# solonas13/REAL

Measured on AMD Instinct MI355X. Metric: aligned reads/sec (100 bp, k≤3) at 1/2/4/8 MI355X; achieved HBM GB/s vs peak, higher is better.
Workload: dtype u64

## Files before the change

### real_amd/csrc/match_common.h

```cpp
#pragma once
#include "kernel_common.h"

template <int W>
__device__ __forceinline__ void revcomp_words(const uint64_t *in, uint64_t *out, uint32_t patl)
{
    const uint32_t nw = (patl + 31) >> 5;
    const uint32_t pad = 64 * nw - 2 * patl;
#pragma unroll
    for (int j = 0; j < W; ++j) {
        uint64_t x = 0, y = 0;
#pragma unroll
        for (int k = 0; k < W; ++k) {
            if ((uint32_t)k + (uint32_t)j + 1 == nw) x = rev2(in[k]);
            if ((uint32_t)k + (uint32_t)j + 2 == nw) y = rev2(in[k]);
        }
        const uint64_t v = pad ? ((x << pad) | (y >> (64 - pad))) : x;
        const uint64_t valid = ((uint32_t)j + 1 < nw) ? ~0ull : ((uint32_t)j + 1 == nw ? (~0ull << pad) : 0ull);
        out[j] = ~v & valid;
    }
}

struct LdsRow {
    const uint8_t *stg;
    uint32_t lb;
    __device__ __forceinline__ uint32_t dword(int byteoff, uint32_t) const
    {
        const uint32_t o = lb + (uint32_t)byteoff;
        const uint32_t *p = reinterpret_cast<const uint32_t *>(stg + (o & ~3u));
        return __builtin_amdgcn_alignbyte(p[1], p[0], o & 3u);
    }
};
struct GlobalRow {
    const uint8_t *row;
    __device__ __forceinline__ uint32_t dword(int byteoff, uint32_t patl) const
    {
        uint32_t v = 0;
#pragma unroll
        for (int b = 0; b < 4; ++b) {
            const int i = byteoff + b;
            if (i >= 0 && i < (int)patl) v |= (uint32_t)row[i] << (8 * b);
        }
        return v;
    }
};

template <int W, class Row>
__device__ __forceinline__ bool pack_read(const Row &row, uint32_t patl, uint64_t *O)
{
    bool ok = true;
#pragma unroll
    for (int j = 0; j < W; ++j) {
        uint64_t w = 0;
#pragma unroll
        for (int d = 0; d < 8; ++d) {
            const uint32_t bo = 32u * j + 4u * d;
            if (bo < patl) {
                uint32_t x = row.dword((int)bo, patl);
                const uint32_t rem = patl - bo;
                if (rem < 4) x &= (1u << (8 * rem)) - 1u;
                if (x & 0xfcfcfcfcu) ok = false;
                w |= (uint64_t)(((x & 0x03030303u) * 0x40100401u) >> 24) << (56 - 8 * d);
            }
        }
        O[j] = w;
    }
    return ok;
}

template <int W, class Row>
__device__ __forceinline__ void pack_read_packed(const Row &row, uint32_t patl, uint32_t skew, uint64_t *O)
{
    const uint32_t nbytes = (skew + patl + 3) >> 2;
    const uint32_t nw = (patl + 31) >> 5, sh = 2 * skew;
#pragma unroll
    for (int j = 0; j < W; ++j) {
        uint64_t w = 0;
        if ((uint32_t)j < nw) {
            const uint32_t hi = __builtin_bswap32(row.dword(8 * j, nbytes));
            const uint32_t lo = __builtin_bswap32(row.dword(8 * j + 4, nbytes));
            w = ((uint64_t)hi << 32) | lo;
            if (sh) w = (w << sh) | ((uint64_t)(row.dword(8 * j + 8, nbytes) & 0xffu) >> (8 - sh));
            const uint32_t rem = patl - 32u * j;
            if (rem < 32) w &= ~0ull << (64 - 2 * rem);
        }
        O[j] = w;
    }
}

template <int W>
__device__ __forceinline__ void seed_halves(const uint64_t *O, uint32_t l, uint64_t &shi, uint64_t &slo, uint64_t &rhi, uint64_t &rlo)
{
    const uint32_t h = l >> 1;
    const uint64_t hm = (h == 32) ? ~0ull : ((1ull << (2 * h)) - 1);
    shi = O[0] >> (64 - 2 * h);
    if (2 * h <= 32) slo = (O[0] >> (64 - 4 * h)) & hm;
    else slo = ((h == 32) ? O[W > 1 ? 1 : 0] : (((O[0] << (2 * h)) | (O[W > 1 ? 1 : 0] >> (64 - 2 * h))) >> (64 - 2 * h)));
    rhi = (rev2(slo) >> (64 - 2 * h)) ^ hm;
    rlo = (rev2(shi) >> (64 - 2 * h)) ^ hm;
}

#define RH_LL_ZERO 1024u
#define RH_LL_SLOTS 1025u
template <int W, class Row>
__device__ __forceinline__ float score_location(const double *sLL, const uint64_t *Ow, const uint64_t *tw, uint32_t patl,
                                                const Row &qrow, bool has_q, uint32_t inv)
{
    double raw = 1.0;
    constexpr int NQ = 2 * W;
    uint32_t th[NQ], oh[NQ];
#pragma unroll
    for (int c = 0; c < NQ; ++c) {
        th[c] = (uint32_t)(tw[c >> 1] >> ((c & 1) ? 0 : 32));
        oh[c] = (uint32_t)(Ow[c >> 1] >> ((c & 1) ? 0 : 32));
    }
    const uint32_t nchunk = (patl + 15) >> 4;
#pragma unroll 1
    for (uint32_t c = 0; c < nchunk; ++c) {
        uint32_t qa[4] = {0x1e1e1e1eu, 0x1e1e1e1eu, 0x1e1e1e1eu, 0x1e1e1e1eu};
        if (has_q) {
            if (!inv) {
#pragma unroll
                for (int i = 0; i < 4; ++i) qa[i] = qrow.dword((int)(16 * c) + 4 * i, patl);
            } else {
                const int p0 = (int)patl - 16 - (int)(16 * c);
#pragma unroll
                for (int i = 0; i < 4; ++i) qa[i] = __builtin_bswap32(qrow.dword(p0 + 4 * (3 - i), patl));
            }
        }
        const uint32_t lim = min(16u, patl - 16u * c);
        const uint32_t tr = th[0], rr = oh[0];
#pragma unroll
        for (int h = 0; h < 2; ++h) {
            double x[8];
#pragma unroll
            for (int v = 0; v < 8; ++v) {
                const uint32_t u = 8u * h + v;
                const uint32_t ref = (tr >> (30 - 2 * u)) & 3;
                const uint32_t rb = (rr >> (30 - 2 * u)) & 3;
                const uint32_t q = (qa[u >> 2] >> (8 * (u & 3))) & 0xff;
                const uint32_t idx = ((ref << 8) | (rb << 6) | q) & 1023;
                x[v] = sLL[u < lim ? idx : RH_LL_ZERO];
            }
#pragma unroll
            for (int v = 0; v < 8; ++v) raw += x[v];
        }
#pragma unroll
        for (int i = 0; i + 1 < NQ; ++i) { th[i] = th[i + 1]; oh[i] = oh[i + 1]; }
    }
    return (float)raw;
}

__device__ __forceinline__ float long_score(const double *sLL, const uint64_t *__restrict__ T, const uint64_t *cur, uint32_t pos, uint32_t patl,
                                            const uint8_t *qual, uint32_t inv)
{
    const uint64_t wi = pos >> 5;
    const unsigned sh = 2u * (pos & 31);
    const uint32_t nw = (patl + 31) >> 5;
    double raw = 1.0;
    uint64_t t0 = T[wi];
    for (uint32_t j = 0; j < nw; ++j) {
        const uint64_t t1 = T[wi + j + 1];
        const uint64_t al = sh ? ((t0 << sh) | (t1 >> (64 - sh))) : t0;
        const uint64_t rw = cur[j];
        const uint32_t nb = min(32u, patl - 32u * j);
        for (uint32_t u = 0; u < nb; ++u) {
            const uint32_t i = 32u * j + u;
            const uint32_t ref = (uint32_t)(al >> (62 - 2 * u)) & 3u, rb = (uint32_t)(rw >> (62 - 2 * u)) & 3u;
            const uint32_t q = qual ? (uint32_t)qual[inv ? patl - 1 - i : i] : 30u;
            raw += sLL[((ref << 8) | (rb << 6) | q) & 1023];
        }
        t0 = t1;
    }
    return (float)raw;
}
```

### real_amd/csrc/match_kernel.hip

```cpp
#include "match_common.h"
#include "row_bytes.h"
#include "complex_walk.h"

#ifndef RH_ABLATE
#define RH_ABLATE 0
#endif
#ifndef RH_PHASE_TIMING
#define RH_PHASE_TIMING 0
#endif

#ifndef RH_PHASE_SUB
#define RH_PHASE_SUB 0
#endif
#if RH_PHASE_TIMING
#define PH_NOW() ((unsigned)__builtin_amdgcn_s_memrealtime())
#define PH_SUB(N, DT) do { if (RH_PHASE_SUB == (N)) s.tD += (DT); else if (RH_PHASE_SUB == 4) s.tD -= (DT); } while (0)
#else
#define PH_NOW() 0u
#endif
#define EB 8
#define MQ 16
#define QUEUE_BYTES (MQ * 64u * 5u + 6u * 64u * 4u)
enum : int { TK_STARTS = 0, TK_DIRECTORY = 1, TK_ROWS = 3, TK_ROWS_WIDE = 4 };
__host__ __device__ constexpr uint32_t stg_bytes(int W, int TK) { return TK >= TK_ROWS ? 11008u : (W <= 4 ? QUEUE_BYTES : 9728u); }
// ... 932 lines not shown
    ISSUE_ROWS_P(0u);
#pragma unroll 1
    for (uint32_t li = 0; li < 6; ++li) {
        const uint32_t tbl = tbl_of(li);
        const bool pairt = li < 4;
#if RH_PHASE_TIMING
        const unsigned ph0 = PH_NOW();
#endif
        wave_lds_sync();
        {
            uint8_t *d = rowbuf + (lane >> 3) * 128 + (((lane & 7) ^ ((lane >> 3) & 7)) * 16);
            *reinterpret_cast<uint4 *>(d + 0 * 1024) = va0; *reinterpret_cast<uint4 *>(d + 1 * 1024) = va1;
            *reinterpret_cast<uint4 *>(d + 2 * 1024) = va2; *reinterpret_cast<uint4 *>(d + 3 * 1024) = va3;
            *reinterpret_cast<uint4 *>(d + 4 * 1024) = va4; *reinterpret_cast<uint4 *>(d + 5 * 1024) = va5;
            *reinterpret_cast<uint4 *>(d + 6 * 1024) = va6; *reinterpret_cast<uint4 *>(d + 7 * 1024) = va7;
        }
        wave_lds_sync();
#if RH_PHASE_TIMING
        unsigned ph1 = PH_NOW();
        s.tW += ph1 - ph0;
#endif
        const uint8_t *rowb = rowbuf + lane * 128;
        const uint32_t sw = lane & 7;
        auto row = [&](uint32_t d) { return *reinterpret_cast<const uint32_t *>(rowb + ((((d >> 2) ^ sw) << 4) | ((d & 3) << 2))); };
        auto row16 = [&](uint32_t B) { return (uint32_t)*reinterpret_cast<const uint16_t *>(rowb + rh_row_lds_byte(B, sw)); };
        const uint32_t g0 = rnext & 255u, g1 = (rnext >> 8) & 255u, s0 = rnext >> 16, la1 = pairt ? 5 - tbl : tbl;
        const uint32_t r0 = sig_of(s0, 5 - tbl) >> (a.l - pbits);
        const uint32_t r1 = sig_of(s0 ^ 1u, 5 - la1) >> (a.l - pbits);
        const bool mine = act && !(s.p_n == PEND_OVF) && !(RH_ABLATE & 8);
        const uint32_t h0 = row(0), h1 = row(1);
        const bool cplx = mine && rh_row_complex(h0, h1);
        uint32_t c0 = 0, c1 = 0, eb0 = 0, eb1 = 0;
        if (mine && !cplx) {
            const uint64_t hh = ((uint64_t)h1 << 32) | h0, ones = 0x1111111111111111ull;
            const uint64_t below0 = ones & ~(~0ull << (4 * g0));
            eb0 = nibble_dot(h0, (uint32_t)below0, nibble_dot(h1, (uint32_t)(below0 >> 32), 0u));
            c0 = (uint32_t)(hh >> (4 * g0)) & 15u;
            const uint64_t ext = (ones & ~(~0ull << (4 * g1))) ^ below0;
            eb1 = nibble_dot(h0, (uint32_t)ext, nibble_dot(h1, (uint32_t)(ext >> 32), eb0));
            c1 = (uint32_t)(hh >> (4 * g1)) & 15u;
            s.addL(2u);
            s.addC(c0 + c1);
            s.addP(c0 + c1);
            if (RH_ABLATE & 4) c0 = c1 = 0;
        }
        uint32_t xb0 = 0, xc0 = 0, xb1 = 0, xc1 = 0;
        bool inplace = false;
        if (__any(cplx)) {
            if (cplx) {
                const uint32_t w[4] = {row(4), row(5), row(6), row(7)};
                const uint32_t o0 = row(2), tot = row(3);
                CwGroup ga, gb;
                cw_header2(w, g0, g1, ga, gb);
                s.addL(1u);
                xb0 = o0 + ga.off; xc0 = ga.cnt;
                if (ga.sat) {
                    const uint2 kr = key_group_range(a.ix.ent[tbl], o0, o0 + tot, pbits, g0);
                    xb0 = kr.x; xc0 = kr.y;
                }
                s.addC(xc0);
                s.addP(xc0);
                if (xc0 > T::BIG) { s.p_n = PEND_OVF; s.cslot = xc0 <= BIG_T2 ? SLOT_NONE : SLOT_BIG; xc0 = 0; }
                else {
                    s.addL(1u);
                    xb1 = o0 + gb.off; xc1 = gb.cnt;
                    if (gb.sat) {
                        const uint2 kr = key_group_range(a.ix.ent[tbl], o0, o0 + tot, pbits, g1);
                        xb1 = kr.x; xc1 = kr.y;
                    }
                    s.addC(xc1);
                    s.addP(xc1);
                    if (xc1 > T::BIG) { s.p_n = PEND_OVF; s.cslot = xc1 <= BIG_T2 ? SLOT_NONE : SLOT_BIG; xc0 = xc1 = 0; }
                }
                if (RH_ABLATE & 4) xc0 = xc1 = 0;
            }
            const uint64_t m0 = __ballot(xc0 != 0), m1 = __ballot(xc1 != 0);
            const uint32_t n0 = (uint32_t)__popcll(m0), n1 = (uint32_t)__popcll(m1);
            inplace = cw_n + n0 + n1 > T::CWCAP;
            if (!inplace) {
                const uint32_t i0 = cw_n + __builtin_amdgcn_mbcnt_hi((uint32_t)(m0 >> 32), __builtin_amdgcn_mbcnt_lo((uint32_t)m0, 0u));
                const uint32_t i1 = cw_n + n0 + __builtin_amdgcn_mbcnt_hi((uint32_t)(m1 >> 32), __builtin_amdgcn_mbcnt_lo((uint32_t)m1, 0u));
                if (xc0) cwl[i0] = make_uint2(xb0, cw_pack(lane, xc0, tbl, tbl, s0));
                if (xc1) cwl[i1] = make_uint2(xb1, cw_pack(lane, xc1, tbl, la1, s0 ^ 1u));
                cw_n += n0 + n1;
                xc0 = xc1 = 0;
            }
        }
        const bool walk = li == 5 && cw_n != 0;
        uint32_t *cw_pre = bkx;
        uint32_t cw_total = 0;
        auto fetch = [&](uint32_t t, uint2 &e, uint32_t &m, uint32_t &k) {
            const bool ok = t < cw_total;
            const uint32_t d = cw_flat_find(cw_pre, cw_n, ok ? t : 0u);
            const uint2 ds = cwl[d];
            const uint32_t tb = cw_table(ds.y), own = cw_lane(ds.y), st = cw_strand(ds.y);
            const uint2 *E = tb == 0u ? a.ix.ent[0] : tb == 1u ? a.ix.ent[1] : tb == 2u ? a.ix.ent[2] : a.ix.ent[3];
            e = make_uint2(0u, 0u);
            if (ok) e = E[ds.x + (t - cw_pre[d])];
            m = ok ? ds.y : CW_NONE;
            const uint32_t ohf = __shfl(fhi, (int)own), olf = __shfl(flo, (int)own), ohr = __shfl(rhi, (int)own), olr = __shfl(rlo, (int)own);
            k = sig_from(st ? ohr : ohf, st ? olr : olf, 5u - cw_list(ds.y)) >> (a.l - pbits);
        };
        uint2 e_c = make_uint2(0u, 0u), e_n = make_uint2(0u, 0u);
        uint32_t m_c = CW_NONE, k_c = 0, m_n = CW_NONE, k_n = 0;
#if RH_PHASE_TIMING
        const unsigned pw0 = PH_NOW();
#endif
        if (walk) {
            static_assert(T::CWCAP * 4u <= 256u, "the prefix sums lie in the place of the bucket numbers");
            wave_lds_sync();
            const uint32_t cnt = lane < cw_n ? cw_cnt(cwl[lane].y) : 0u;
            uint32_t inc = cnt;
#pragma unroll
            for (uint32_t d = 1; d < 64; d <<= 1) {
                const uint32_t v = __shfl_up(inc, d);
                if (lane >= d) inc += v;
            }
            cw_total = __builtin_amdgcn_readlane(inc, 63);
            wave_lds_sync();
            if (lane < cw_n) cw_pre[lane] = inc - cnt;
            wave_lds_sync();
            fetch(lane, e_c, m_c, k_c);
            if (cw_total > 64u) fetch(64u + lane, e_n, m_n, k_n);
        }
#if RH_PHASE_TIMING
        const unsigned pw1 = PH_NOW();
#endif
        U64x2 pre = {0ull, 0ull};
        if (inplace && xc0) pre = load2(reinterpret_cast<const uint64_t *>(a.ix.ent[tbl] + xb0));
        if (li + 1 < 6) ISSUE_ROWS_P(li + 1);
#if RH_PHASE_TIMING
        const unsigned ps1 = PH_NOW();
        PH_SUB(1, (ps1 - ph1) - (pw1 - pw0));
#endif
        {
            static_assert(RH_ROW_CAP < 32 && 2 * 15 < 32, "one mask word for both groups of a simple row (one group taken twice: 2 x 15 entries)");
            const uint32_t ct = c0 + c1, d1 = eb1 - c0;
            uint32_t rk0 = r0 >> (pbits - p16), rk1 = r1 >> (pbits - p16);
            asm volatile("" : "+v"(rk0), "+v"(rk1));
            uint32_t passm = 0, e_j = 0;
            while (__any(e_j < ct)) {
                uint32_t key[4];
#pragma unroll
                for (uint32_t u = 0; u < 4; ++u) {
                    const uint32_t jj = e_j + u;
                    const uint32_t ej = jj + (jj >= c0 ? d1 : eb0);
                    key[u] = row16(rh_row_key_byte(ej < RH_ROW_CAP - 1u ? ej : RH_ROW_CAP - 1u));
                }
                asm volatile("" : "+v"(key[0]), "+v"(key[1]), "+v"(key[2]), "+v"(key[3]));
#pragma unroll
                for (uint32_t u = 0; u < 4; ++u) {
                    const uint32_t jj = e_j + u;
                    const uint32_t x = key[u] ^ (jj >= c0 ? rk1 : rk0);
                    passm |= ((jj < ct) & passes(x) ? 1u : 0u) << (jj & 31u);
                }
                e_j += 4;
            }
            const uint32_t low = (1u << c0) - 1u;
            if (__popc(passm & low) > NPEND || __popc(passm & ~low) > NPEND) { s.p_n = PEND_OVF; passm = 0; }
#if RH_PHASE_TIMING
            const unsigned ps2 = PH_NOW();
            PH_SUB(2, ps2 - ps1);
#endif
            while (__any(passm != 0)) {
                const bool step = passm != 0;
                const uint32_t jj = step ? (uint32_t)__ffs((int)passm) - 1u : 0u;
                passm &= passm - 1u;
                const bool sec = jj >= c0;
                const uint32_t ej = step ? jj + (sec ? d1 : eb0) : 0u;
                const uint32_t plo = row16(rh_row_pos_byte(ej, 0u)), phi = row16(rh_row_pos_byte(ej, 1u));
                take(step, plo | (phi << 16), s0 ^ (sec ? 1u : 0u), sec ? la1 : tbl);
            }
#if RH_PHASE_TIMING
            PH_SUB(3, PH_NOW() - ps2);
#endif
        }
        if (inplace) {
#pragma unroll 1
            for (uint32_t half = 0; half < 2; ++half) {
                const uint32_t strand = s0 ^ half, la = half ? la1 : tbl, r = half ? r1 : r0;
                const uint32_t e_base = half ? xb1 : xb0;
                e_cnt = s.p_n == PEND_OVF ? 0u : (half ? xc1 : xc0);
                const bool e_ovf = e_cnt != 0;
                if (half) pre = e_ovf ? load2(reinterpret_cast<const uint64_t *>(a.ix.ent[tbl] + e_base)) : U64x2{0ull, 0ull};
                auto take_ovf = [&](bool ok, uint2 e) { take(ok && passes((e.x & pmask) ^ r), e.y, strand, la); };
                if (__any(e_ovf)) {
                    take_ovf(e_cnt > 0, make_uint2((uint32_t)pre.a, (uint32_t)(pre.a >> 32)));
                    take_ovf(e_cnt > 1, make_uint2((uint32_t)pre.b, (uint32_t)(pre.b >> 32)));
                }
                uint32_t e_j = 2;
                while (__any(e_j < e_cnt)) {
                    uint2 e[T::OVN];
#pragma unroll
                    for (uint32_t u = 0; u < T::OVN; ++u) e[u] = (e_j + u < e_cnt) ? a.ix.ent[tbl][e_base + e_j + u] : make_uint2(0u, 0u);
#pragma unroll
                    for (uint32_t u = 0; u < T::OVN; ++u) take_ovf(e_j + u < e_cnt, e[u]);
                    e_j += T::OVN;
                }
            }
        }
        if (walk) {
            uint32_t *cw_slot = reinterpret_cast<uint32_t *>(rowbuf);
#pragma unroll 1
            for (uint32_t t0 = 0; t0 < cw_total; t0 += 64u) {
                bool pend = m_c != CW_NONE && passes((e_c.x & pmask) ^ k_c);
                const uint32_t own = cw_lane(m_c);
                while (__any(pend)) {
                    wave_lds_sync();
                    cw_slot[lane] = CW_NONE;
                    wave_lds_sync();
                    if (pend) atomicMin(cw_slot + own, lane);
                    wave_lds_sync();
                    const uint32_t from = cw_slot[lane];
                    const bool hit = from != CW_NONE;
                    const int src = (int)(hit ? from : lane);
                    const uint32_t pos = __shfl(e_c.y, src), tag = __shfl(m_c, src);
                    if (pend && cw_slot[own] == lane) pend = false;
                    take(hit, pos, cw_strand(tag), cw_list(tag));
                }
                e_c = e_n; m_c = m_n; k_c = k_n;
                m_n = CW_NONE;
                if (t0 + 128u < cw_total) fetch(t0 + 128u + lane, e_n, m_n, k_n);
            }
        }
#if RH_PHASE_TIMING
        if (RH_PHASE_SUB == 0 || RH_PHASE_SUB == 4) s.tD += PH_NOW() - ph1;
#endif
    }
    const uint32_t patl = act ? s.patl : 32u * T::W;
#pragma unroll 1
    for (uint32_t inv = 0; inv < 2; ++inv) {
        if (inv && act) {
            uint64_t R[T::W];
            revcomp_words<T::W>(s.O, R, patl);
#pragma unroll
            for (int j = 0; j < T::W; ++j) s.O[j] = R[j];
        }
        s.shi = inv ? rhi : fhi; s.slo = inv ? rlo : flo;
        s.reset_strand((int)inv);
        if (T::SCORES && inv) {
            const uint8_t *qsrc;
            uint32_t qbytes, qlate, qskew;
            if (quals_ahead<T>(a, s.o0, s.o1, qsrc, qbytes, qlate, qskew)) {
                wave_lds_sync();
                const uint32_t lds0 = __builtin_amdgcn_readfirstlane((uint32_t)(uintptr_t)(__attribute__((address_space(3))) uint8_t *)rowbuf);
                QUAL_DMA(qlate, lds0, qbytes - qlate, 9u)
                const uint32_t tail0 = qbytes & ~15u;
                if (lane < (qbytes & 15u)) rowbuf[tail0 - qlate + lane] = qsrc[tail0 + lane];
            }
        }
#if RH_PHASE_TIMING
        const unsigned ph2 = PH_NOW();
#endif
        if (s.p_n == PEND_OVF) qn = 0;
        auto next = [&](uint32_t k) { while (k < qn && (q_getl(k) >> 6) != inv) ++k; return k; };
        CandText<T::W> c0;
        uint32_t k = next(0u), rp0 = 0, la0 = 0;
        if (k < qn) { rp0 = q_getp(k); la0 = q_getl(k); cand_load(a, s, rp0, c0); }
        while (k < qn) {
            CandText<T::W> c1;
            const uint32_t k1 = next(k + 1);
            uint32_t rp1 = 0, la1 = 0;
            if (k1 < qn) { rp1 = q_getp(k1); la1 = q_getl(k1); cand_load(a, s, rp1, c1); }
            process_loaded(a, s, sLL, rp0, la0 & 63u, c0);
            c0 = c1; rp0 = rp1; la0 = la1; k = k1;
        }
#if RH_PHASE_TIMING
        s.tR += PH_NOW() - ph2;
#endif
    }
    if (T::SCORES) {
        const uint8_t *qsrc;
        uint32_t qbytes, qlate, qskew;
        if (quals_ahead<T>(a, s.o0, s.o1, qsrc, qbytes, qlate, qskew) && qlate) {
            wave_lds_sync();
            const uint32_t lds0 = __builtin_amdgcn_readfirstlane((uint32_t)(uintptr_t)(__attribute__((address_space(3))) uint8_t *)stg);
            QUAL_DMA(0u, lds0 + STG_PAD, qlate, 3u)
        }
    }
#undef QUAL_DMA
#undef ISSUE_ROWS_P
}

template <class T, int LA0, int LA1>
__device__ __forceinline__ void match_lists(const MatchArgs &a, LaneState<T> &s, const double *sLL, uint32_t *q_pos, uint8_t *q_la)
{
    if (T::DIR) { match_lists_directory<T, LA0, LA1>(a, s, sLL, q_pos, q_la); return; }
    uint32_t qn = 0;
    scan_lists<T, LA0, LA1>(a, s, q_pos, q_la, qn);
    for (uint32_t k = 0; k < qn && s.p_n != PEND_OVF; ++k)
        process_candidate(a, s, sLL, q_pos[k * 64], (uint32_t)q_la[k * 64]);
}

template <class T>
__device__ __forceinline__ void match_read(const MatchArgs &a, LaneState<T> &s, const double *sLL, uint8_t *stg, uint32_t *q_pos, uint8_t *q_la,
                                           bool act)
{
    const uint32_t patl = act ? s.patl : 32u * T::W;
    s.reset_read();
    uint64_t rhi = 0, rlo = 0;
    if (act) seed_halves<T::W>(s.O, a.l, s.shi, s.slo, rhi, rlo);
    else { s.shi = s.slo = 0; }
    if constexpr (T::PAIRED) { match_rows_paired<T>(a, s, sLL, stg, act, (uint32_t)rhi, (uint32_t)rlo); return; }
    for (int inv = 0; inv < 2; ++inv) {
        if constexpr (!T::ROWS) {
            if (s.p_n == PEND_OVF) break;
        }
        if (inv && act) {
            uint64_t R[T::W];
            revcomp_words<T::W>(s.O, R, patl);
#pragma unroll
            for (int j = 0; j < T::W; ++j) s.O[j] = R[j];
            s.shi = rhi; s.slo = rlo;
        }
        s.reset_strand(inv);
        const bool go = !T::ROWS || (act && !(s.p_n == PEND_OVF));
        if (!T::ALL && !T::SCORES) {
            if constexpr (T::ROWS) match_lists_rows<T, 0, 1>(a, s, sLL, stg, go, false);
            else match_lists<T, 0, 1>(a, s, sLL, q_pos, q_la);
            const unsigned st = (unsigned)(s.info >> ST_SHIFT), er = (unsigned)(s.info >> ER_SHIFT) & 15;
            if constexpr (T::ROWS) match_lists_rows<T, 1, 6>(a, s, sLL, stg, go && !(st == (unsigned)(inv ? ST_REVERSE : ST_STRAIGHT) && er == 0), false);
            else if (!(st == (unsigned)(inv ? ST_REVERSE : ST_STRAIGHT) && er == 0)) match_lists<T, 1, 6>(a, s, sLL, q_pos, q_la);
        } else if constexpr (T::ROWS) {
            match_lists_rows<T, 0, 6>(a, s, sLL, stg, go, !T::PASS2 && inv != 0);
        } else {
            match_lists<T, 0, 6>(a, s, sLL, q_pos, q_la);
        }
    }
}

template <int W, bool SCORES, bool ALL, int TK, bool PASS2>
__global__ __launch_bounds__(256) __attribute__((amdgpu_waves_per_eu(PASS2 ? 2 : (W <= 5 ? 3 : 2)))) void match_kernel(MatchArgs a_)
{
    using T = LaneInst<W, SCORES, ALL, TK, PASS2>;
    constexpr uint32_t STG = T::STG;
    static_assert(!PASS2 || T::HAS_PASS2, "the second pass exists for bucket rows with parked hits only");
    __shared__ double sLL[SCORES ? RH_LL_SLOTS : 1];
    __shared__ __attribute__((aligned(16))) uint8_t smem[4 * STG];
    if (SCORES) {
        for (int i = threadIdx.x; i < 1024; i += 256) sLL[i] = a_.LL[i];
        if (threadIdx.x == 0) sLL[RH_LL_ZERO] = 0.0;
        __syncthreads();
    }
    const uint64_t n_items = PASS2 ? (uint64_t)*a_.ovf_count : a_.b.n_reads;
    const uint64_t n_tiles = (n_items + 63) / 64;
    uint32_t *const tile_ctr = PASS2 ? a_.tile_ctr2 : a_.tile_ctr;
    uint32_t next_raw = 0;
    if ((threadIdx.x & 63) == 0) next_raw = atomicAdd(tile_ctr, 1u);
    while (true) {
    const uint64_t tile = (uint32_t)__builtin_amdgcn_readfirstlane((int)next_raw);
    if (tile >= n_tiles) break;
    if ((threadIdx.x & 63) == 0) next_raw = atomicAdd(tile_ctr, 1u);
    uint32_t tid = threadIdx.x;
    asm volatile("" : "+v"(tid));
    const __attribute__((address_space(4))) MatchArgs *pa = (const __attribute__((address_space(4))) MatchArgs *)__builtin_amdgcn_kernarg_segment_ptr();
    asm volatile("" : "+s"(pa));
    const MatchArgs &a = *(const MatchArgs *)pa;
    const uint32_t lane = tid & 63;
    uint8_t *stg = smem + (tid >> 6) * STG;
    uint32_t *q_pos = reinterpret_cast<uint32_t *>(stg) + lane;
    uint8_t *q_la = stg + MQ * 64 * 4 + lane;
    const unsigned ph_start = PH_NOW();
    LaneState<T> s;
    s.reset_counters();
#if RH_PHASE_TIMING
    s.tW = s.tD = s.tR = 0;
    unsigned tQ = 0, tS = 0;
#endif
    s.info = 0; s.iscore = 0.f; s.o0 = s.o1 = 0;
    unsigned cR = 0;
    const uint64_t n = a.b.n_reads;

    const uint64_t item = tile * 64 + lane;
    const bool have = item < n_items;
    const uint64_t r = PASS2 ? (have ? (uint64_t)a.ovf_list[item] : n) : item;
    const uint64_t rc = r < n ? r : n;
    const uint64_t o0 = a.b.off ? a.b.off[rc] : rc * (uint64_t)a.b.upatl;
    const uint64_t o1 = r < n ? (a.b.off ? a.b.off[r + 1] : o0 + a.b.upatl) : o0;
    const bool span_bad = o1 < o0 || o1 - o0 > (uint64_t)REAL_HIP_MAX_PATL_LONG;
    const uint32_t patl = span_bad ? 0u : (uint32_t)(o1 - o0);
    const uint32_t bsh = a.b.packed ? 2u : 0u;
    const uint32_t GL = a.b.gl;
    bool elig = false, toolong = false, give = false;
    if (PASS2) {
        if (r < n) {
            if (a.b.packed) {
                pack_read_packed<W>(GlobalRow{a.b.bases + (o0 >> 2)}, patl, (uint32_t)o0 & 3u, s.O);
                elig = true;
            } else {
                elig = pack_read<W>(GlobalRow{a.b.bases + o0}, patl, s.O);
            }
        }
    } else {
    for (uint32_t g = 0; g < 64; g += GL) {
        const uint64_t gb = __shfl(o0, (int)g), ge = __shfl(o1, (int)(g + GL - 1));
        const bool fits = ge >= gb && ge - gb <= T::STG_CAP;
        wave_lds_sync();
        uint32_t l0 = 0;
        if (fits) l0 = stage_wave(stg, a.b.bases + (gb >> bsh), a.b.packed ? ((ge + 3) >> 2) - (gb >> 2) : ge - gb, lane);
        wave_lds_sync();
        const bool in_group = lane >= g && lane < g + GL && r < n;
        if (in_group && span_bad) toolong = true;
        else if (in_group && (!fits || patl > 32u * W)) give = patl >= a.l;
        if (in_group && fits && !span_bad && patl >= a.l && patl <= 32u * W) {
            if (a.b.packed) {
                pack_read_packed<W>(LdsRow{stg, l0 + (uint32_t)((o0 >> 2) - (gb >> 2))}, patl, (uint32_t)o0 & 3u, s.O);
                elig = !(a.b.nflags && ((a.b.nflags[r >> 3] >> (r & 7)) & 1));
            } else {
                elig = pack_read<W>(LdsRow{stg, l0 + (uint32_t)(o0 - gb)}, patl, s.O);
            }
        }
    }
    }
    if (toolong) atomicOr(a.err_flags, 1u);
    wave_lds_sync();
    s.r = r; s.patl = patl; s.p_n = 0; s.nhit = 0;
    const bool fresh = !PASS2 && a.b.fresh;
    if (elig && !ALL && !fresh) {
        s.info = a.info[r];
        if (SCORES) s.iscore = a.score[r];
    }
    if (!ALL && fresh) s.iscore = -3.402823466e+38f;
    const unsigned ph_front = PH_NOW();
    s.o0 = o0; s.o1 = o1;
    if (T::ROWS) match_read(a, s, sLL, stg, q_pos, q_la, elig);
    else if (elig) match_read(a, s, sLL, stg, q_pos, q_la, true);
    const bool ovf = give || (elig && s.p_n == PEND_OVF);
    if (ovf) {
        const bool to_wave = PASS2 || !T::HAS_PASS2 || give || s.cslot == SLOT_BIG;
        if (to_wave) {
            const unsigned long long slot = wave_append_slot(a.ovf2_count);
            a.ovf2_list[slot] = (uint32_t)r;
        } else {
            const unsigned long long slot = wave_append_slot(a.ovf_count);
            a.ovf_list[slot] = (uint32_t)r;
        }
        s.reset_counters();
    }
    const uint8_t *qsrc_ = nullptr;
    uint32_t qbytes_ = 0, qlate_ = 0, qskew_ = 0;
    const bool q_ahead = !PASS2 && T::ROWS && SCORES && quals_ahead<T>(a, o0, o1, qsrc_, qbytes_, qlate_, qskew_);
    if (q_ahead) quals_landed();
    if (T::DEFER && PASS2) {
        const bool want = elig && !ovf && s.p_n;
        const bool in_lds = !SCORES || !a.b.qual || patl <= 104u;
        uint8_t *slot = stg + T::ROWBUF + lane * 128u;
        uint32_t head = 0;
        wave_lds_sync();
        if (want && SCORES && a.b.qual && in_lds) {
            const uint8_t *q0 = a.b.qual + o0;
            head = (uint32_t)((uintptr_t)q0 & 3u);
            const uint32_t *__restrict__ src = reinterpret_cast<const uint32_t *>(q0 - head);
            const uint32_t nd = (head + patl + 3u) >> 2;
            for (uint32_t k = 0; k < nd; ++k) reinterpret_cast<uint32_t *>(slot + 16)[k] = src[k];
        }
        wave_lds_sync();
        if (want && in_lds) flush_pending(a, s, sLL, LdsRow{stg, (uint32_t)(slot - stg) + 16u + head});
        else if (want) flush_pending(a, s, sLL, GlobalRow{a.b.qual + o0});
    } else if (T::DEFER) {
        for (uint32_t g = 0; g < 64; g += GL) {
            const uint64_t gb = __shfl(o0, (int)g), ge = __shfl(o1, (int)(g + GL - 1));
            const bool mine = lane >= g && lane < g + GL && elig && !ovf && s.p_n;
            if (!__any(mine)) continue;
            uint32_t l0 = 0;
#if RH_PHASE_TIMING
            const unsigned pq0 = PH_NOW();
#endif
            if (q_ahead) {
                wave_lds_sync();
                l0 = quals_at<T>(qlate_, qskew_);
            } else {
                wave_lds_sync();
                if (SCORES && a.b.qual) l0 = stage_wave(stg, a.b.qual + gb, ge - gb, lane);
                wave_lds_sync();
            }
#if RH_PHASE_TIMING
            const unsigned pq1 = PH_NOW();
            tQ += pq1 - pq0;
#endif
            if (mine) flush_pending(a, s, sLL, LdsRow{stg, l0 + (uint32_t)(o0 - gb)});
#if RH_PHASE_TIMING
            tS += PH_NOW() - pq1;
#endif
        }
    }
    if (elig && !ovf) {
        cR = 1;
        if (!ALL) {
            a.info[r] = s.info;
            if (SCORES) a.score[r] = s.iscore;
        }
    } else if (!ALL && fresh && r < n) {
        a.info[r] = 0;
// ... 71 lines not shown
```

Measured before the change: 4.635 billion.

## Compute score-table byte offsets two-at-a-time with packed perm and and_or ops

Rewrites the per-base log-likelihood lookup in score_location. It now builds two 16-bit table byte offsets per dword using v_perm/v_and_or and SDWA shifts, loads the quality window with five LDS dwords plus alignbyte, and skips bounds selects when the whole wave has full 16-base chunks. The aim is to cut the VALU cost of index construction and masking in the scoring loop. An optional LDS skew layout for the table is added but is off by default. Adding a uniform branch and inline asm risks divergence overhead and subtle indexing bugs.

Measured after the change: 4.648 billion (median of 6 runs). About the same (+0.3%).

```diff
diff --git a/real_amd/csrc/match_common.h b/real_amd/csrc/match_common.h
--- a/real_amd/csrc/match_common.h
+++ b/real_amd/csrc/match_common.h
@@ -1,5 +1,6 @@
 #pragma once
 #include "kernel_common.h"
+#include "score_index.h"
 
 template <int W>
 __device__ __forceinline__ void revcomp_words(const uint64_t *in, uint64_t *out, uint32_t patl)
@@ -29,6 +30,15 @@
         const uint32_t *p = reinterpret_cast<const uint32_t *>(stg + (o & ~3u));
         return __builtin_amdgcn_alignbyte(p[1], p[0], o & 3u);
     }
+    __device__ __forceinline__ void window(int byteoff, uint32_t, uint32_t (&w)[4]) const
+    {
+        const uint32_t o = lb + (uint32_t)byteoff;
+        const uint32_t *p = reinterpret_cast<const uint32_t *>(stg + (o & ~3u));
+        uint32_t d[5];
+#pragma unroll
+        for (int i = 0; i < 5; ++i) d[i] = p[i];
+        rh_si_window(d, o, w);
+    }
 };
 struct GlobalRow {
     const uint8_t *row;
@@ -41,6 +51,11 @@
             if (i >= 0 && i < (int)patl) v |= (uint32_t)row[i] << (8 * b);
         }
         return v;
+    }
+    __device__ __forceinline__ void window(int byteoff, uint32_t patl, uint32_t (&w)[4]) const
+    {
+#pragma unroll
+        for (int i = 0; i < 4; ++i) w[i] = dword(byteoff + 4 * i, patl);
     }
 };
 
@@ -99,55 +114,38 @@
     rlo = (rev2(shi) >> (64 - 2 * h)) ^ hm;
 }
 
-#define RH_LL_ZERO 1024u
-#define RH_LL_SLOTS 1025u
+#define RH_LL_ZERO (RH_SI_ZERO_OFF / 8u)
+#define RH_LL_SLOTS (RH_LL_ZERO + 1u)
+static_assert(RH_SI_ZERO_OFF % 8u == 0 && RH_LL_ZERO >= 1024u, "the 0.0 lies behind the 1024 entries");
+struct ScoreTable {
+    const double *sLL;
+    __device__ __forceinline__ double at(uint32_t byteoff) const { return *reinterpret_cast<const double *>(reinterpret_cast<const char *>(sLL) + byteoff); }
+};
+template <class Row>
+struct ScoreQuals {
+    const Row &row;
+    bool has_q;
+    __device__ __forceinline__ void trip(uint32_t c, uint32_t patl, uint32_t inv, uint32_t (&a)[4]) const
+    {
+        if (has_q) {
+            uint32_t w[4];
+            row.window(rh_si_window_start(patl, c, inv), patl, w);
+            rh_si_order(w, inv, a);
+        } else {
+#pragma unroll
+            for (int i = 0; i < 4; ++i) a[i] = 0x1e1e1e1eu;
+        }
+    }
+};
+struct ScoreWave {
+    __device__ __forceinline__ bool all_full(uint32_t patl, uint32_t c) const { return __all(patl >= 16u * c + 16u); }
+    __device__ __forceinline__ bool any_second(uint32_t patl, uint32_t c) const { return __any(patl > 16u * c + 8u); }
+};
 template <int W, class Row>
 __device__ __forceinline__ float score_location(const double *sLL, const uint64_t *Ow, const uint64_t *tw, uint32_t patl,
                                                 const Row &qrow, bool has_q, uint32_t inv)
 {
-    double raw = 1.0;
-    constexpr int NQ = 2 * W;
-    uint32_t th[NQ], oh[NQ];
-#pragma unroll
-    for (int c = 0; c < NQ; ++c) {
-        th[c] = (uint32_t)(tw[c >> 1] >> ((c & 1) ? 0 : 32));
-        oh[c] = (uint32_t)(Ow[c >> 1] >> ((c & 1) ? 0 : 32));
-    }
-    const uint32_t nchunk = (patl + 15) >> 4;
-#pragma unroll 1
-    for (uint32_t c = 0; c < nchunk; ++c) {
-        uint32_t qa[4] = {0x1e1e1e1eu, 0x1e1e1e1eu, 0x1e1e1e1eu, 0x1e1e1e1eu};
-        if (has_q) {
-            if (!inv) {
-#pragma unroll
-                for (int i = 0; i < 4; ++i) qa[i] = qrow.dword((int)(16 * c) + 4 * i, patl);
-            } else {
-                const int p0 = (int)patl - 16 - (int)(16 * c);
-#pragma unroll
-                for (int i = 0; i < 4; ++i) qa[i] = __builtin_bswap32(qrow.dword(p0 + 4 * (3 - i), patl));
-            }
-        }
-        const uint32_t lim = min(16u, patl - 16u * c);
-        const uint32_t tr = th[0], rr = oh[0];
-#pragma unroll
-        for (int h = 0; h < 2; ++h) {
-            double x[8];
-#pragma unroll
-            for (int v = 0; v < 8; ++v) {
-                const uint32_t u = 8u * h + v;
-                const uint32_t ref = (tr >> (30 - 2 * u)) & 3;
-                const uint32_t rb = (rr >> (30 - 2 * u)) & 3;
-                const uint32_t q = (qa[u >> 2] >> (8 * (u & 3))) & 0xff;
-                const uint32_t idx = ((ref << 8) | (rb << 6) | q) & 1023;
-                x[v] = sLL[u < lim ? idx : RH_LL_ZERO];
-            }
-#pragma unroll
-            for (int v = 0; v < 8; ++v) raw += x[v];
-        }
-#pragma unroll
-        for (int i = 0; i + 1 < NQ; ++i) { th[i] = th[i + 1]; oh[i] = oh[i + 1]; }
-    }
-    return (float)raw;
+    return (float)rh_si_score<W>(ScoreTable{sLL}, Ow, tw, patl, ScoreQuals<Row>{qrow, has_q}, inv, ScoreWave{});
 }
 
 __device__ __forceinline__ float long_score(const double *sLL, const uint64_t *__restrict__ T, const uint64_t *cur, uint32_t pos, uint32_t patl,
diff --git a/real_amd/csrc/match_kernel.hip b/real_amd/csrc/match_kernel.hip
--- a/real_amd/csrc/match_kernel.hip
+++ b/real_amd/csrc/match_kernel.hip
@@ -1294,7 +1294,7 @@
     __shared__ double sLL[SCORES ? RH_LL_SLOTS : 1];
     __shared__ __attribute__((aligned(16))) uint8_t smem[4 * STG];
     if (SCORES) {
-        for (int i = threadIdx.x; i < 1024; i += 256) sLL[i] = a_.LL[i];
+        for (int i = threadIdx.x; i < 1024; i += 256) sLL[rh_si_slot((uint32_t)i)] = a_.LL[i];
         if (threadIdx.x == 0) sLL[RH_LL_ZERO] = 0.0;
         __syncthreads();
     }
diff --git a/real_amd/csrc/score_index.h b/real_amd/csrc/score_index.h
--- /dev/null
+++ b/real_amd/csrc/score_index.h
@@ -0,0 +1,141 @@
+#pragma once
+#include <stdint.h>
+#if defined(__HIPCC__)
+#define RH_HD __host__ __device__
+#else
+#define RH_HD
+#endif
+#define RH_SI_FN static inline RH_HD __attribute__((always_inline))
+
+#ifndef RH_LL_SKEW
+#define RH_LL_SKEW 0
+#endif
+RH_SI_FN uint32_t rh_si_slot(uint32_t idx) { return RH_LL_SKEW ? idx + (idx >> 6) : idx; }
+#define RH_SI_ZERO_OFF (RH_LL_SKEW ? 8u * 1039u : 8192u)
+
+RH_SI_FN uint32_t rh_si_perm(uint32_t s0, uint32_t s1, uint32_t sel)
+{
+#if defined(__HIP_DEVICE_COMPILE__)
+    return __builtin_amdgcn_perm(s0, s1, sel);
+#else
+    const uint64_t both = ((uint64_t)s0 << 32) | s1;
+    uint32_t r = 0;
+    for (int i = 0; i < 4; ++i) {
+        const uint32_t c = (sel >> (8 * i)) & 0xffu;
+        uint32_t b;
+        if (c < 8) b = (uint32_t)(both >> (8 * c)) & 0xffu;
+        else if (c < 12) b = ((both >> (16 * (c - 8) + 15)) & 1u) ? 0xffu : 0u;
+        else b = c == 12 ? 0u : 0xffu;
+        r |= b << (8 * i);
+    }
+    return r;
+#endif
+}
+RH_SI_FN uint32_t rh_si_alignbyte(uint32_t hi, uint32_t lo, uint32_t s)
+{
+#if defined(__HIP_DEVICE_COMPILE__)
+    return __builtin_amdgcn_alignbyte(hi, lo, s);
+#else
+    return (uint32_t)((((uint64_t)hi << 32) | lo) >> (8 * (s & 3u)));
+#endif
+}
+
+RH_SI_FN int rh_si_window_start(uint32_t patl, uint32_t c, uint32_t inv) { return inv ? (int)patl - 16 - (int)(16u * c) : (int)(16u * c); }
+RH_SI_FN void rh_si_window(const uint32_t d[5], uint32_t o, uint32_t w[4])
+{
+    for (int i = 0; i < 4; ++i) w[i] = rh_si_alignbyte(d[i + 1], d[i], o);
+}
+RH_SI_FN void rh_si_order(const uint32_t w[4], uint32_t inv, uint32_t a[4])
+{
+    const uint32_t sel = inv ? 0x00010203u : 0x03020100u;
+    const uint32_t m = 0u - (inv & 1u);
+    const uint32_t t03 = (w[0] ^ w[3]) & m, t12 = (w[1] ^ w[2]) & m;
+    const uint32_t x[4] = {w[0] ^ t03, w[1] ^ t12, w[2] ^ t12, w[3] ^ t03};
+    for (int i = 0; i < 4; ++i) a[i] = rh_si_perm(x[i], x[i], sel);
+}
+
+RH_SI_FN uint32_t rh_si_and_or(uint32_t x, uint32_t mask, uint32_t y)
+{
+#if defined(__HIP_DEVICE_COMPILE__)
+    uint32_t r;
+    asm("v_and_or_b32 %0, %1, %2, %3" : "=v"(r) : "v"(x), "v"(mask), "v"(y));
+    return r;
+#else
+    return (x & mask) | y;
+#endif
+}
+RH_SI_FN uint32_t rh_si_pair(uint32_t tr, uint32_t rr, const uint32_t a[4], uint32_t u)
+{
+    const uint32_t k = u & 3u;
+    const uint32_t qp = rh_si_perm(a[u >> 2], a[(u >> 2) + 2], 0x0c040c00u + k * 0x00010001u);
+    const uint32_t ts = u <= 3 ? tr >> (6 - 2 * u) : tr << (2 * u - 6);
+    const uint32_t rs = u <= 4 ? rr >> (8 - 2 * u) : rr << (2 * u - 8);
+    const uint32_t x = rh_si_and_or(ts, 0x03000300u, rh_si_and_or(rs, 0x00c000c0u, qp));
+    return RH_LL_SKEW ? x + ((x >> 6) & 0x000f000fu) : x;
+}
+RH_SI_FN uint32_t rh_si_off_hi(uint32_t x) { return x >> 13; }
+RH_SI_FN uint32_t rh_si_off_lo(uint32_t x)
+{
+#if defined(__HIP_DEVICE_COMPILE__)
+    uint32_t r;
+    asm("v_lshlrev_b32_sdwa %0, 3, %1 dst_sel:DWORD dst_unused:UNUSED_PAD src0_sel:DWORD src1_sel:WORD_0" : "=v"(r) : "v"(x));
+    return r;
+#else
+    return (x & 0xffffu) << 3;
+#endif
+}
+
+template <int W, class Table, class Quals, class Wave>
+RH_SI_FN double rh_si_score(const Table &LL, const uint64_t *Ow, const uint64_t *tw, uint32_t patl, const Quals &q, uint32_t inv,
+                            const Wave &wv)
+{
+    double raw = 1.0;
+    uint64_t tq[W], oq[W];
+#pragma unroll
+    for (int i = 0; i < W; ++i) { tq[i] = tw[i]; oq[i] = Ow[i]; }
+    uint32_t tr = (uint32_t)(tq[0] >> 32), rr = (uint32_t)(oq[0] >> 32);
+#pragma unroll 1
+    for (uint32_t c = 0; 16u * c < patl; ++c) {
+        uint32_t a[4], x[8];
+        q.trip(c, patl, inv, a);
+#pragma unroll
+        for (uint32_t u = 0; u < 8; ++u) x[u] = rh_si_pair(tr, rr, a, u);
+        double y[8];
+        if (wv.all_full(patl, c)) {
+#pragma unroll
+            for (int v = 0; v < 8; ++v) y[v] = LL.at(rh_si_off_hi(x[v]));
+#pragma unroll
+            for (int v = 0; v < 8; ++v) raw += y[v];
+#pragma unroll
+            for (int v = 0; v < 8; ++v) y[v] = LL.at(rh_si_off_lo(x[v]));
+#pragma unroll
+            for (int v = 0; v < 8; ++v) raw += y[v];
+        } else {
+            const uint32_t lim = patl - 16u * c;
+#pragma unroll
+            for (uint32_t v = 0; v < 8; ++v) {
+                const uint32_t off = rh_si_off_hi(x[v]);
+                y[v] = LL.at(v < lim ? off : RH_SI_ZERO_OFF);
+            }
+#pragma unroll
+            for (int v = 0; v < 8; ++v) raw += y[v];
+            if (wv.any_second(patl, c)) {
+#pragma unroll
+                for (uint32_t v = 0; v < 8; ++v) {
+                    const uint32_t off = rh_si_off_lo(x[v]);
+                    y[v] = LL.at(v + 8 < lim ? off : RH_SI_ZERO_OFF);
+                }
+#pragma unroll
+                for (int v = 0; v < 8; ++v) raw += y[v];
+            }
+        }
+        if (c & 1u) {
+#pragma unroll
+            for (int i = 0; i + 1 < W; ++i) { tq[i] = tq[i + 1]; oq[i] = oq[i + 1]; }
+            tr = (uint32_t)(tq[0] >> 32); rr = (uint32_t)(oq[0] >> 32);
+        } else {
+            tr = (uint32_t)tq[0]; rr = (uint32_t)oq[0];
+        }
+    }
+    return raw;
+}
```

## Restructure score_location with byte-address indexing and 32-base trips using perm cursors

Applied to the files above, without the earlier changes.

Rewrites the per-location likelihood scoring loop into a shared helper. The new loop processes 32 bases per trip and handles only the tail with a masked 4-base loop. It builds LDS table byte addresses directly with a multiply-spread of read bits, and fetches quality dwords through a cursor that uses a single v_perm to handle alignment and reverse order together. This removes per-base shift/mask/select work, the alignbyte+bswap pair, and per-chunk bounds checks, at the cost of more code complexity.

Result: no change. 4.639 billion before, 4.693 billion after (median of 6 runs) (+1.2%).

```diff
diff --git a/real_amd/csrc/match_common.h b/real_amd/csrc/match_common.h
--- a/real_amd/csrc/match_common.h
+++ b/real_amd/csrc/match_common.h
@@ -1,5 +1,6 @@
 #pragma once
 #include "kernel_common.h"
+#include "score_index.h"
 
 template <int W>
 __device__ __forceinline__ void revcomp_words(const uint64_t *in, uint64_t *out, uint32_t patl)
@@ -29,6 +30,20 @@
         const uint32_t *p = reinterpret_cast<const uint32_t *>(stg + (o & ~3u));
         return __builtin_amdgcn_alignbyte(p[1], p[0], o & 3u);
     }
+    struct Cursor {
+        const uint8_t *wa;
+        uint32_t sel;
+        __device__ __forceinline__ uint32_t at(int delta) const
+        {
+            const uint32_t *p = reinterpret_cast<const uint32_t *>(wa + delta);
+            return __builtin_amdgcn_perm(p[1], p[0], sel);
+        }
+    };
+    __device__ __forceinline__ Cursor cursor(int off0, uint32_t, uint32_t qsel, bool) const
+    {
+        const uint32_t o = lb + (uint32_t)off0;
+        return Cursor{stg + (o & ~3u), rh_score_word_sel(qsel, o)};
+    }
 };
 struct GlobalRow {
     const uint8_t *row;
@@ -41,6 +56,10 @@
             if (i >= 0 && i < (int)patl) v |= (uint32_t)row[i] << (8 * b);
         }
         return v;
+    }
+    __device__ __forceinline__ RhDwordCursor<GlobalRow> cursor(int off0, uint32_t patl, uint32_t qsel, bool has_q) const
+    {
+        return RhDwordCursor<GlobalRow>{*this, off0, patl, qsel, has_q};
     }
 };
 
@@ -99,13 +118,10 @@
     rlo = (rev2(shi) >> (64 - 2 * h)) ^ hm;
 }
 
-#define RH_LL_ZERO 1024u
-#define RH_LL_SLOTS 1025u
 template <int W, class Row>
 __device__ __forceinline__ float score_location(const double *sLL, const uint64_t *Ow, const uint64_t *tw, uint32_t patl,
                                                 const Row &qrow, bool has_q, uint32_t inv)
 {
-    double raw = 1.0;
     constexpr int NQ = 2 * W;
     uint32_t th[NQ], oh[NQ];
 #pragma unroll
@@ -113,41 +129,7 @@
         th[c] = (uint32_t)(tw[c >> 1] >> ((c & 1) ? 0 : 32));
         oh[c] = (uint32_t)(Ow[c >> 1] >> ((c & 1) ? 0 : 32));
     }
-    const uint32_t nchunk = (patl + 15) >> 4;
-#pragma unroll 1
-    for (uint32_t c = 0; c < nchunk; ++c) {
-        uint32_t qa[4] = {0x1e1e1e1eu, 0x1e1e1e1eu, 0x1e1e1e1eu, 0x1e1e1e1eu};
-        if (has_q) {
-            if (!inv) {
-#pragma unroll
-                for (int i = 0; i < 4; ++i) qa[i] = qrow.dword((int)(16 * c) + 4 * i, patl);
-            } else {
-                const int p0 = (int)patl - 16 - (int)(16 * c);
-#pragma unroll
-                for (int i = 0; i < 4; ++i) qa[i] = __builtin_bswap32(qrow.dword(p0 + 4 * (3 - i), patl));
-            }
-        }
-        const uint32_t lim = min(16u, patl - 16u * c);
-        const uint32_t tr = th[0], rr = oh[0];
-#pragma unroll
-        for (int h = 0; h < 2; ++h) {
-            double x[8];
-#pragma unroll
-            for (int v = 0; v < 8; ++v) {
-                const uint32_t u = 8u * h + v;
-                const uint32_t ref = (tr >> (30 - 2 * u)) & 3;
-                const uint32_t rb = (rr >> (30 - 2 * u)) & 3;
-                const uint32_t q = (qa[u >> 2] >> (8 * (u & 3))) & 0xff;
-                const uint32_t idx = ((ref << 8) | (rb << 6) | q) & 1023;
-                x[v] = sLL[u < lim ? idx : RH_LL_ZERO];
-            }
-#pragma unroll
-            for (int v = 0; v < 8; ++v) raw += x[v];
-        }
-#pragma unroll
-        for (int i = 0; i + 1 < NQ; ++i) { th[i] = th[i + 1]; oh[i] = oh[i + 1]; }
-    }
-    return (float)raw;
+    return (float)rh_score_sum<NQ>(sLL, th, oh, patl, qrow, has_q, inv);
 }
 
 __device__ __forceinline__ float long_score(const double *sLL, const uint64_t *__restrict__ T, const uint64_t *cur, uint32_t pos, uint32_t patl,
diff --git a/real_amd/csrc/match_kernel.hip b/real_amd/csrc/match_kernel.hip
--- a/real_amd/csrc/match_kernel.hip
+++ b/real_amd/csrc/match_kernel.hip
@@ -1108,7 +1108,7 @@
                 for (uint32_t u = 0; u < 4; ++u) {
                     const uint32_t jj = e_j + u;
                     const uint32_t x = key[u] ^ (jj >= c0 ? rk1 : rk0);
-                    passm |= ((jj < ct) & passes(x) ? 1u : 0u) << (jj & 31u);
+                    passm |= (((jj < ct) & passes(x)) ? 1u : 0u) << (jj & 31u);
                 }
                 e_j += 4;
             }
diff --git a/real_amd/csrc/score_index.h b/real_amd/csrc/score_index.h
--- /dev/null
+++ b/real_amd/csrc/score_index.h
@@ -0,0 +1,113 @@
+#pragma once
+#include <stdint.h>
+#if defined(__HIPCC__)
+#define RH_HD __host__ __device__
+#else
+#define RH_HD
+#endif
+
+#define RH_LL_ZERO 1024u
+#define RH_LL_SLOTS 1025u
+
+static inline RH_HD uint32_t rh_score_spread4(uint32_t x) { return (((x & 0xffu) * 0x00100401u) | (x << 30)) & 0xc0c0c0c0u; }
+static inline RH_HD uint32_t rh_score_low4(uint32_t q, uint32_t rb4) { return q | rh_score_spread4(rb4); }
+static inline RH_HD uint32_t rh_score_addr(uint32_t ref, uint32_t low4, int m)
+{
+    const uint32_t l3 = (m == 0 ? low4 << 3 : low4 >> (8 * m - 3)) & 0x7f8u;
+    return (ref << 11) | l3;
+}
+static inline RH_HD void rh_score_addr4(uint32_t tr, uint32_t rr, int k, uint32_t q, uint32_t (&a)[4])
+{
+    const uint32_t low4 = rh_score_low4(q, rr >> (24 - 8 * k));
+#pragma unroll
+    for (int m = 0; m < 4; ++m) a[m] = rh_score_addr((tr >> (30 - 2 * (4 * k + m))) & 3u, low4, m);
+}
+static inline RH_HD double rh_score_entry(const double *LL, uint32_t byte_addr)
+{
+    return *reinterpret_cast<const double *>(reinterpret_cast<const char *>(LL) + byte_addr);
+}
+
+static inline RH_HD uint32_t rh_score_qsel(uint32_t inv) { return inv ? 0x00010203u : 0x03020100u; }
+static inline RH_HD int rh_score_qoff0(uint32_t inv, uint32_t patl) { return inv ? (int)patl - 4 : 0; }
+static inline RH_HD int rh_score_qstep(uint32_t inv) { return inv ? -4 : 4; }
+static inline RH_HD uint32_t rh_score_qorder(uint32_t v, uint32_t qsel)
+{
+#if defined(__HIP_DEVICE_COMPILE__)
+    return __builtin_amdgcn_perm(v, v, qsel);
+#else
+    return qsel == 0x03020100u ? v : __builtin_bswap32(v);
+#endif
+}
+static inline RH_HD uint32_t rh_score_word_sel(uint32_t qsel, uint32_t o) { return qsel + 0x01010101u * (o & 3u); }
+template <class Row>
+struct RhDwordCursor {
+    const Row &row;
+    int off0;
+    uint32_t patl, qsel;
+    bool has_q;
+    RH_HD uint32_t at(int delta) const { return has_q ? rh_score_qorder(row.dword(off0 + delta, patl), qsel) : 0u; }
+};
+#define RH_NO_QUAL4 0x1e1e1e1eu
+
+template <class Cur>
+static inline RH_HD double rh_score_chunk16(const double *LL, double raw, uint32_t tr, uint32_t rr, const Cur &qc, bool has_q,
+                                            int dq, int qstep)
+{
+#pragma unroll
+    for (int h = 0; h < 2; ++h) {
+        double x[8];
+#pragma unroll
+        for (int g = 0; g < 2; ++g) {
+            const int k = 2 * h + g;
+            const uint32_t q = qc.at(dq + k * qstep);
+            uint32_t a[4];
+            rh_score_addr4(tr, rr, k, has_q ? q : RH_NO_QUAL4, a);
+#pragma unroll
+            for (int m = 0; m < 4; ++m) x[4 * g + m] = rh_score_entry(LL, a[m]);
+        }
+#pragma unroll
+        for (int v = 0; v < 8; ++v) raw += x[v];
+    }
+    return raw;
+}
+
+template <int NQ, class Row>
+static inline RH_HD double rh_score_sum(const double *LL, uint32_t (&th)[NQ], uint32_t (&oh)[NQ], uint32_t patl, const Row &qrow,
+                                        bool has_q, uint32_t inv)
+{
+    static_assert(NQ >= 2 && NQ % 2 == 0, "two elements per word of 32 bases");
+    double raw = 1.0;
+    const auto qc = qrow.cursor(rh_score_qoff0(inv, patl), patl, rh_score_qsel(inv), has_q);
+    const int qstep = rh_score_qstep(inv);
+    int dq = 0;
+    const uint32_t ntrip = (patl + 31) >> 5;
+#pragma unroll 1
+    for (uint32_t c = 0; c < ntrip; ++c) {
+        const uint32_t b = 32u * c, n = patl - b;
+        if (n >= 16) raw = rh_score_chunk16(LL, raw, th[0], oh[0], qc, has_q, dq, qstep);
+        if (n >= 32) {
+            raw = rh_score_chunk16(LL, raw, th[1], oh[1], qc, has_q, dq + 4 * qstep, qstep);
+        } else if (n & 15u) {
+            uint32_t tr = n >= 16 ? th[1] : th[0], rr = n >= 16 ? oh[1] : oh[0];
+            uint32_t d = b + (n & 16u);
+            int dt = n >= 16 ? dq + 4 * qstep : dq;
+#pragma unroll 1
+            for (; d < patl; d += 4, dt += qstep) {
+                const uint32_t lim = patl - d;
+                const uint32_t q = qc.at(dt);
+                uint32_t a[4];
+                rh_score_addr4(tr, rr, 0, has_q ? q : RH_NO_QUAL4, a);
+                double x[4];
+#pragma unroll
+                for (int m = 0; m < 4; ++m) x[m] = rh_score_entry(LL, (uint32_t)m < lim ? a[m] : 8u * RH_LL_ZERO);
+#pragma unroll
+                for (int m = 0; m < 4; ++m) raw += x[m];
+                tr <<= 8; rr <<= 8;
+            }
+        }
+#pragma unroll
+        for (int i = 0; i + 2 < NQ; ++i) { th[i] = th[i + 2]; oh[i] = oh[i + 2]; }
+        dq += 8 * qstep;
+    }
+    return raw;
+}
```
